# NICTA/revrand

Measured on AMD Instinct MI355X. Metric: feature-rows/sec (Phi + PhiT Phi + PhiT y) at N=10M D=32 F=4096, higher is better.
Workload: dtype f32; 1 GPU; RandomRBF nbases=2048 (F=4096), D=32, N=10000000 f32, features + MFMA Gram, rows sharded over 1 GPU(s); rows_per_gpu=10000000, device=(gfx950:sramecc+:xnack-), gram_engine=f32

## Files before the change

revrand_amd/csrc/rr_rff.hip:

```cpp
#include "rr_syrk_args.h"
#include <algorithm>
#include <map>
#include <mutex>
#include <type_traits>




__device__ __forceinline__ void sincos_rev(float t, float &s, float &c) {
    const float f = t - __builtin_rintf(t);
    s = __builtin_amdgcn_sinf(f);
    c = __builtin_amdgcn_cosf(f);
}

__device__ __forceinline__ void sincos_rev(double t, double &s, double &c) { rr_sincos_rev_f64(t, s, c); }
typedef double doublex4 __attribute__((ext_vector_type(4)));

template <int DMAX, bool GUARD, typename TX, typename TC>
__device__ __forceinline__ TC project_row(const TX *__restrict__ xr, int d, const TC (&w)[DMAX]) {
    TC z = 0;
#pragma unroll
    for (int i = 0; i < DMAX; ++i) {
        if (!GUARD || i < d) z = fma((TC)xr[i], w[i], z);
    }
// ... 970 lines not shown
        syrk_diag_body<4>(p, lds, wave, lane);
}

typedef float floatx4 __attribute__((ext_vector_type(4)));

template <int OFF>
__device__ __forceinline__ float lds_read_b32_off(unsigned addr) {
    float r;
    asm volatile("ds_read_b32 %0, %1 offset:%2" : "=v"(r) : "v"(addr), "i"(OFF));
    return r;
}

template <int NB, int ED>
struct KOpsD16 {
    float2v a[NB], b[NB];
    float x0, x1;
    template <int P>
    __device__ __forceinline__ void load(const unsigned (&abase)[NB], const unsigned (&bbase)[NB], unsigned xbase) {
#pragma unroll
        for (int e = 0; e < NB; ++e)
            if (e != ED) a[e] = lds_read2st64<16 * P, 16 * P + 8>(abase[e]);
#pragma unroll
        for (int e = 0; e < NB; ++e)
            if (e != ED) b[e] = lds_read2st64<16 * P, 16 * P + 8>(bbase[e]);
        x0 = lds_read_b32_off<4096 * P>(xbase);
        x1 = lds_read_b32_off<4096 * P + 64>(xbase);
    }
};

template <int NB, int ED, int FIRST, int LAST>
__device__ __forceinline__ void gram_mfma_d16(const KOpsD16<NB, ED> &o, floatx16 (&acc)[NB], floatx4 (&dd)[3]) {
#pragma unroll
    for (int q = FIRST; q < LAST; ++q) {
        if (q < NB - 1 || q >= NB + 2) {
            const int s_ = q < NB - 1 ? 0 : 1;
            const int r_ = q < NB - 1 ? q : q - (NB + 2);
            const int e = r_ < ED ? r_ : r_ + 1;
            acc[e] = __builtin_amdgcn_mfma_f32_32x32x2f32(o.a[e][s_], o.b[e][s_], acc[e], 0, 0, 0);
        } else {
            const int t = q - (NB - 1);
            dd[t] = __builtin_amdgcn_mfma_f32_16x16x4f32(t == 2 ? o.x1 : o.x0, t == 0 ? o.x0 : o.x1, dd[t], 0, 0, 0);
        }
    }
}

#define RR_PAIRD16(P, CUR, NXT)                                \
    lds_wait();                                                \
    __builtin_amdgcn_sched_barrier(0);                         \
    gram_mfma_d16<NB, ED, 0, 1>(CUR, acc, dd);                 \
    __builtin_amdgcn_sched_barrier(0);                         \
    if ((P) + 1 < KB / 4) NXT.template load<((P) + 1) & (KB / 4 - 1)>(abase, bbase, xbase); \
    __builtin_amdgcn_sched_barrier(0);                         \
    gram_mfma_d16<NB, ED, 1, 2 * NB + 1>(CUR, acc, dd);        \
    __builtin_amdgcn_sched_barrier(0);

template <int NB, int ED, int KB>
__device__ __forceinline__ void syrk_diag16_body(const SyrkArgs &p, float *lds, int wave, int lane, const unsigned bid) {
    const int ta = bid % p.nb;
    const int ks = bid / p.nb;
    const int ca = ta * GR_TC;
    const int64_t row_begin = (int64_t)ks * p.rows_per_split;
    int64_t row_end = row_begin + p.rows_per_split;
    if (row_end > p.rows) row_end = p.rows;

    const unsigned lds0 = (unsigned)(size_t)(__attribute__((address_space(3))) float *)lds;
    const unsigned lane_off = 4u * ((lane >> 5) * GR_TC + (lane & 31));
    int bi[NB], bj[NB];
#pragma unroll
    for (int e = 0; e < NB; ++e) {
        bi[e] = RR_DIAG_I[wave][e];
        bj[e] = RR_DIAG_J[wave][e];
    }
    RR_DEV_ASSERT(bi[ED] == bj[ED]);
    const unsigned lane_off16 = 4u * ((lane >> 4) * GR_TC + 32 * bi[ED] + (lane & 15));
    floatx16 acc[NB];
    floatx4 dd[3];
#pragma unroll
    for (int e = 0; e < NB; ++e)
#pragma unroll
        for (int k = 0; k < 16; ++k) acc[e][k] = 0.f;
#pragma unroll
    for (int t = 0; t < 3; ++t) dd[t] = floatx4{0.f, 0.f, 0.f, 0.f};

    const unsigned voff = 16u * lane, ldp4 = (unsigned)p.ldp * 4u;
    auto dma_tile = [&](float *buf, int64_t kb0) {
        RR_DEV_ASSERT(kb0 + KB <= p.rows && ca + GR_TC <= p.ldp && p.rows % KB == 0 && p.rows_per_split % KB == 0);
        const rr_rsrc_t ra = rr_make_rsrc(p.P + kb0 * p.ldp + ca, 0x7fffffffu);
#pragma unroll
        for (int k = 0; k < KB / 8; ++k) {
            const int lr = (KB / 8) * wave + k;
            __builtin_amdgcn_raw_ptr_buffer_load_lds(ra, (lptr_t)(buf + lr * GR_TC), 16, voff, (unsigned)lr * ldp4, 0, 0);
        }
    };

    const int64_t nkb = (row_end - row_begin) / KB;
    if (nkb > 0) {
        dma_tile(lds, row_begin);
        __syncthreads();
        for (int64_t kb = 0; kb < nkb; ++kb) {
            const int cbuf = (int)(kb & 1);
            const int slot = p.spread ? rr_dma_slot(wave, p.spread) : 0;
            auto dma_next = [&]() {
                if (kb + 1 < nkb) dma_tile(lds + (cbuf ^ 1) * (KB * GR_TC), row_begin + (kb + 1) * KB);
            };
            if (slot == 0) dma_next();
            unsigned abase[NB], bbase[NB];
#pragma unroll
            for (int e = 0; e < NB; ++e) {
                abase[e] = lds0 + cbuf * (4u * KB * GR_TC) + lane_off + 128u * bi[e];
                bbase[e] = lds0 + cbuf * (4u * KB * GR_TC) + lane_off + 128u * bj[e];
            }
            const unsigned xbase = lds0 + cbuf * (4u * KB * GR_TC) + lane_off16;
            KOpsD16<NB, ED> o0, o1;
            o0.template load<0>(abase, bbase, xbase);
            RR_PAIRD16(0, o0, o1)
            if (slot == 1) dma_next();
            RR_PAIRD16(1, o1, o0)
            if (slot == 2) dma_next();
            RR_PAIRD16(2, o0, o1)
            if (slot == 3) dma_next();
            RR_PAIRD16(3, o1, o0)
            RR_PAIRD16(4, o0, o1) RR_PAIRD16(5, o1, o0) RR_PAIRD16(6, o0, o1) RR_PAIRD16(7, o1, o0)
            if constexpr (KB == 64) {
                RR_PAIRD16(8, o0, o1) RR_PAIRD16(9, o1, o0) RR_PAIRD16(10, o0, o1) RR_PAIRD16(11, o1, o0)
                RR_PAIRD16(12, o0, o1) RR_PAIRD16(13, o1, o0) RR_PAIRD16(14, o0, o1) RR_PAIRD16(15, o1, o0)
            }
            __syncthreads();
        }
    }

    const int hi = lane >> 5;
#pragma unroll
    for (int e = 0; e < NB; ++e) {
        if (e == ED) continue;
        const int64_t gc = ca + 32 * bj[e] + (lane & 31);
#pragma unroll
        for (int k = 0; k < 16; ++k) {
            const int64_t gr = ca + 32 * bi[e] + (k & 3) + 8 * (k >> 2) + 4 * hi;
            if (gr <= gc) rr_syrk_out(p, ks, gr, gc, acc[e][k]);
        }
    }
#pragma unroll
    for (int t = 0; t < 3; ++t) {
        const int64_t gc = ca + 32 * bi[ED] + (t >= 1 ? 16 : 0) + (lane & 15);
#pragma unroll
        for (int k = 0; k < 4; ++k) {
            const int64_t gr = ca + 32 * bi[ED] + (t == 2 ? 16 : 0) + 4 * (lane >> 4) + k;
            if (gr <= gc) rr_syrk_out(p, ks, gr, gc, dd[t][k]);
        }
    }
}
#undef RR_PAIRD16

template <int KB>
__device__ __forceinline__ void syrk_diag16_dispatch(const SyrkArgs &p, float *lds, const unsigned bid) {
    const int lane = threadIdx.x & 63;
    const int wave = __builtin_amdgcn_readfirstlane(threadIdx.x >> 6);
    switch (wave) {
        case 0: case 1: case 2: case 3: syrk_diag16_body<5, 0, KB>(p, lds, wave, lane, bid); break;
        case 4: syrk_diag16_body<4, 3, KB>(p, lds, wave, lane, bid); break;
        case 5: syrk_diag16_body<4, 2, KB>(p, lds, wave, lane, bid); break;
        case 6: syrk_diag16_body<4, 1, KB>(p, lds, wave, lane, bid); break;
        default: syrk_diag16_body<4, 0, KB>(p, lds, wave, lane, bid); break;
    }
}

template <int KB>
__global__ void __launch_bounds__(GR_THREADS, 2)
rr_syrk_f32_diag16_kernel(const SyrkArgs p) {
    __shared__ float lds[2 * KB * GR_TC];
    syrk_diag16_dispatch<KB>(p, lds, blockIdx.x);
}

constexpr int GS_TC = 128, GS_KB = 32, GS_LD = 2 * GS_TC, GS_THREADS = 256;

__global__ void __launch_bounds__(GS_THREADS, 2)
rr_syrk_f32_small_kernel(const SyrkArgs p) {
    __shared__ __attribute__((aligned(16))) float lds[2][GS_KB * GS_LD];
    const int tid = threadIdx.x, lane = tid & 63, wave = tid >> 6, wr = wave >> 1, wc = wave & 1;
    const int nb = (int)(p.ldp / GS_TC);
    const int64_t ks = blockIdx.x / p.ntiles;
    int t = (int)(blockIdx.x % p.ntiles), ta = 0;
    while (t >= nb - ta) {
        t -= nb - ta;
        ++ta;
    }
    const int tb = ta + t;
    const int64_t ca = (int64_t)ta * GS_TC, cb = (int64_t)tb * GS_TC;
    const int64_t r0 = ks * p.rows_per_split;
    int64_t r1 = r0 + p.rows_per_split;
    if (r1 > p.rows) r1 = p.rows;
    const int nkb = (int)((r1 - r0 + GS_KB - 1) / GS_KB);
    floatx16 acc[2][2];
#pragma unroll
    for (int i = 0; i < 2; ++i)
#pragma unroll
        for (int j = 0; j < 2; ++j)
#pragma unroll
            for (int e = 0; e < 16; ++e) acc[i][j][e] = 0.f;
    const int lr = tid >> 5, lc = tid & 31;
    float4 ra[4], rb[4];
    auto gload = [&](int kb) {
        const float *base = p.P + (r0 + (int64_t)kb * GS_KB + lr) * p.ldp;
#pragma unroll
        for (int u = 0; u < 4; ++u) {
            ra[u] = *(const float4 *)(base + (int64_t)8 * u * p.ldp + ca + 4 * lc);
            rb[u] = *(const float4 *)(base + (int64_t)8 * u * p.ldp + cb + 4 * lc);
        }
    };
    auto lstore = [&](int buf) {
#pragma unroll
        for (int u = 0; u < 4; ++u) {
            *(float4 *)&lds[buf][(lr + 8 * u) * GS_LD + 4 * lc] = ra[u];
            *(float4 *)&lds[buf][(lr + 8 * u) * GS_LD + GS_TC + 4 * lc] = rb[u];
        }
    };
    if (nkb > 0) {
        gload(0);
        lstore(0);
    }
    __syncthreads();
    const int i32 = lane & 31, kk = lane >> 5;
    for (int kb = 0; kb < nkb; ++kb) {
        const int cur = kb & 1;
        if (kb + 1 < nkb) gload(kb + 1);
        const float *L = lds[cur];
#pragma unroll
        for (int k2 = 0; k2 < GS_KB; k2 += 2) {
            const float *row = L + (k2 + kk) * GS_LD;
            const float a0 = row[wr * 64 + i32], a1 = row[wr * 64 + 32 + i32];
            const float b0 = row[GS_TC + wc * 64 + i32], b1 = row[GS_TC + wc * 64 + 32 + i32];
            acc[0][0] = __builtin_amdgcn_mfma_f32_32x32x2f32(a0, b0, acc[0][0], 0, 0, 0);
            acc[0][1] = __builtin_amdgcn_mfma_f32_32x32x2f32(a0, b1, acc[0][1], 0, 0, 0);
            acc[1][0] = __builtin_amdgcn_mfma_f32_32x32x2f32(a1, b0, acc[1][0], 0, 0, 0);
            acc[1][1] = __builtin_amdgcn_mfma_f32_32x32x2f32(a1, b1, acc[1][1], 0, 0, 0);
        }
        if (kb + 1 < nkb) lstore(cur ^ 1);
        __syncthreads();
    }
#pragma unroll
    for (int i = 0; i < 2; ++i)
#pragma unroll
        for (int j = 0; j < 2; ++j) {
            const int64_t gc = cb + wc * 64 + 32 * j + i32;
#pragma unroll
            for (int e = 0; e < 16; ++e) {
                const int64_t gr = ca + wr * 64 + 32 * i + (e & 3) + 8 * (e >> 2) + 4 * kk;
                if (gr <= gc) rr_syrk_out(p, ks, gr, gc, acc[i][j][e]);
            }
        }
}

__global__ void __launch_bounds__(GR_THREADS, 2)
rr_syrk_f32_merged_kernel(const SyrkArgs p, const SyrkArgs pd, const unsigned n_off) {
    __shared__ float lds[2 * GR_KB * GR_LD];
    if (blockIdx.x < n_off) rr_syrk_f32_body<3>(p, lds, blockIdx.x);
    else syrk_diag16_dispatch<32>(pd, lds, blockIdx.x - n_off);
}

constexpr int G64_TC = 128;
constexpr int G64_KB = 16;
constexpr int G64_LDB = 2 * G64_TC * 8 + 128;
constexpr int G64_THREADS = 256;

struct Syrk64Args {
    const double *P;
    int64_t rows, ldp;
    int F, nb, ntiles;
    int64_t rows_per_split;
    double *G;
    int offdiag_only;
    int lower_tri = 0;
    double *part = nullptr;
    int64_t part_stride = 0;
};

__device__ __forceinline__ void rr_syrk64_out(const Syrk64Args &p, int64_t ks, int64_t gr, int64_t gc, double v) {
    if (p.part != nullptr) p.part[ks * p.part_stride + gr * p.ldp + gc] = v;
    else unsafeAtomicAdd(&p.G[gr * (int64_t)p.F + gc], v);
}

template <typename T>
__global__ void __launch_bounds__(256)
rr_syrk_det_reduce_kernel(const T *__restrict__ part, int64_t stride, int64_t ldp, int F, int nsplit, double *__restrict__ G,
                          double *__restrict__ bcol) {
    const int64_t gc = (int64_t)blockIdx.x * 256 + threadIdx.x, gr = blockIdx.y;
    if (gc < gr || gc > F || (gc == F && bcol == nullptr)) return;
    const T *q = part + gr * ldp + gc;
    double s = 0.0;
    for (int k = 0; k < nsplit; ++k) s += (double)q[(int64_t)k * stride];
    if (gc < F) G[gr * (int64_t)F + gc] += s;
    else bcol[gr] += s;
}

template <int OFF>
__device__ __forceinline__ double lds_read_b64(unsigned addr) {
    double r;
    asm volatile("ds_read_b64 %0, %1 offset:%2" : "=v"(r) : "v"(addr), "i"(OFF));
    return r;
}

struct KOps64 {
    double a[4], b[4];
    template <int T>
    __device__ __forceinline__ void load(unsigned abase, unsigned bbase) {
#pragma unroll
        for (int i = 0; i < 4; ++i) a[i] = 0;
        a[0] = lds_read_b64<4 * T * G64_LDB + 0 * 128>(abase);
        a[1] = lds_read_b64<4 * T * G64_LDB + 1 * 128>(abase);
        a[2] = lds_read_b64<4 * T * G64_LDB + 2 * 128>(abase);
        a[3] = lds_read_b64<4 * T * G64_LDB + 3 * 128>(abase);
        b[0] = lds_read_b64<4 * T * G64_LDB + 0 * 128>(bbase);
        b[1] = lds_read_b64<4 * T * G64_LDB + 1 * 128>(bbase);
        b[2] = lds_read_b64<4 * T * G64_LDB + 2 * 128>(bbase);
        b[3] = lds_read_b64<4 * T * G64_LDB + 3 * 128>(bbase);
    }
};

template <int FIRST, int LAST>
__device__ __forceinline__ void gram64_mfma(const KOps64 &o, doublex4 (&acc)[4][4]) {
#pragma unroll
    for (int q = FIRST; q < LAST; ++q)
        acc[q >> 2][q & 3] = __builtin_amdgcn_mfma_f64_16x16x4f64(o.a[q >> 2], o.b[q & 3], acc[q >> 2][q & 3], 0, 0, 0);
}

#define RR_STEP64(T, CUR, NXT)                                  \
    lds_wait();                                                 \
    __builtin_amdgcn_sched_barrier(0);                          \
    gram64_mfma<0, 1>(CUR, acc);                                \
    __builtin_amdgcn_sched_barrier(0);                          \
    if ((T) + 1 < 4) NXT.template load<((T) + 1) & 3>(abase, bbase); \
    __builtin_amdgcn_sched_barrier(0);                          \
    gram64_mfma<1, 16>(CUR, acc);                               \
    __builtin_amdgcn_sched_barrier(0);

__global__ void __launch_bounds__(G64_THREADS, 2)
rr_syrk_f64_kernel(const Syrk64Args p) {
    __shared__ __attribute__((aligned(16))) unsigned char lds[2 * G64_KB * G64_LDB];

    const int tid = threadIdx.x;
    const int lane = tid & 63;
    const int wave = __builtin_amdgcn_readfirstlane(tid >> 6);

    int tdx = blockIdx.x % p.ntiles;
    const int ks = blockIdx.x / p.ntiles;
    int ta = 0;
    const int od = p.offdiag_only;
    while (tdx >= p.nb - ta - od) {
        tdx -= p.nb - ta - od;
        ++ta;
    }
    const int tb = ta + tdx + od;
    const int ca = ta * G64_TC, cb = tb * G64_TC;

    int64_t row_begin = (int64_t)ks * p.rows_per_split;
    int64_t row_end = row_begin + p.rows_per_split;
    if (row_end > p.rows) row_end = p.rows;
    if (p.lower_tri && row_begin < cb) row_begin = cb;
    if (row_begin >= row_end && p.part == nullptr) return;

    const int wr = wave >> 1, wc_ = wave & 1;
    const unsigned lds0 = (unsigned)(size_t)(__attribute__((address_space(3))) unsigned char *)lds;
    const unsigned aoff = (lane >> 4) * G64_LDB + 8u * (wr * 64 + (lane & 15));
    const unsigned boff = (lane >> 4) * G64_LDB + 8u * (G64_TC + wc_ * 64 + (lane & 15));
    doublex4 acc[4][4];
#pragma unroll
    for (int i = 0; i < 4; ++i)
#pragma unroll
        for (int j = 0; j < 4; ++j)
#pragma unroll
            for (int e = 0; e < 4; ++e) acc[i][j][e] = 0.0;

    const unsigned voff = 16u * lane, ldp8 = (unsigned)p.ldp * 8u;
    auto dma_tile = [&](unsigned char *buf, int64_t kb0) {
        const rr_rsrc_t ra = rr_make_rsrc(p.P + kb0 * p.ldp + ca, 0x7fffffffu), rb = rr_make_rsrc(p.P + kb0 * p.ldp + cb, 0x7fffffffu);
#pragma unroll
        for (int k = 0; k < 4; ++k) {
            const int lr = 4 * wave + k;
            unsigned char *dst = buf + lr * G64_LDB;
            __builtin_amdgcn_raw_ptr_buffer_load_lds(ra, (lptr_t)dst, 16, voff, (unsigned)lr * ldp8, 0, 0);
            __builtin_amdgcn_raw_ptr_buffer_load_lds(rb, (lptr_t)(dst + G64_TC * 8), 16, voff, (unsigned)lr * ldp8, 0, 0);
        }
    };

    const int64_t nkb = (row_end - row_begin) / G64_KB;
    RR_DEV_ASSERT(p.rows % G64_KB == 0 && p.rows_per_split % G64_KB == 0 && cb + G64_TC <= p.ldp && row_end <= p.rows);
    if (nkb > 0) {
        dma_tile(lds, row_begin);
        __syncthreads();
        for (int64_t kb = 0; kb < nkb; ++kb) {
            const int cbuf = (int)(kb & 1);
            if (kb + 1 < nkb) dma_tile(lds + (cbuf ^ 1) * (G64_KB * G64_LDB), row_begin + (kb + 1) * G64_KB);
            const unsigned abase = lds0 + cbuf * (G64_KB * G64_LDB) + aoff;
            const unsigned bbase = lds0 + cbuf * (G64_KB * G64_LDB) + boff;
            KOps64 o0, o1;
            o0.load<0>(abase, bbase);
            RR_STEP64(0, o0, o1) RR_STEP64(1, o1, o0) RR_STEP64(2, o0, o1) RR_STEP64(3, o1, o0)
            __syncthreads();
        }
    }

    const int64_t F = p.F;
#pragma unroll
    for (int i = 0; i < 4; ++i)
#pragma unroll
        for (int j = 0; j < 4; ++j) {
            const int64_t gc = cb + wc_ * 64 + j * 16 + (lane & 15);
#pragma unroll
            for (int e = 0; e < 4; ++e) {
                const int64_t gr = ca + wr * 64 + i * 16 + (lane >> 4) + 4 * e;
// ... 877 lines not shown
                part[t1] = y; part[t2] = x;
                cur += d;
                if (cur < best) { best = cur; best_part = part; }
            }
        }
        part = best_part;
    }
    std::vector<int> fill(nxcd, 0);
    for (int t = 0; t < ntiles; ++t) map[(size_t)fill[part[t]]++ * nxcd + part[t]] = t;
}


int rr_launch_syrk_f32(rr_ctx *c, const float *P, int64_t rows, int64_t ldp, int F, double *dG, hipEvent_t mid,
                       double *bcol = nullptr) {
    if (c->gram_engine != 0) {
        RR_REQUIRE(bcol == nullptr, "gram: the rider column needs the f32 engine");
        RR_REQUIRE(!c->deterministic, "gram: deterministic mode (rr_set_deterministic) needs the f32 engine, not a split 16-bit one");
        return rr_launch_syrk_bf16(c, c->gram_engine, P, nullptr, rows, ldp, F, dG, mid);
    }
    RR_REQUIRE(bcol == nullptr || F < ldp, "gram: no pad column for the rider");
    static const bool small_off = getenv("RR_SYRK_SMALL") != nullptr && atoi(getenv("RR_SYRK_SMALL")) == 0;
    const int64_t big_tiles = (ldp / GR_TC) * (ldp / GR_TC + 1) / 2;
    if (!small_off && ldp <= 1024 && big_tiles * ((rows + 1023) / 1024) < c->num_cu && rows % GS_KB == 0 && !getenv("RR_GRAM_ABLATE")) {
        const int nbs = (int)(ldp / GS_TC), nt = nbs * (nbs + 1) / 2;
        int64_t ns = std::max<int64_t>((2 * c->num_cu + nt - 1) / nt, (rows + 32767) / 32768);
        ns = std::min<int64_t>(ns, std::max<int64_t>(rows / 128, 1));
        const int64_t rps_s = ((rows + ns - 1) / ns + GS_KB - 1) / GS_KB * GS_KB;
        ns = (rows + rps_s - 1) / rps_s;
        SyrkArgs a;
        a.P = P; a.rows = rows; a.ldp = ldp; a.F = F; a.nb = nbs; a.ntiles = nt; a.rows_per_split = rps_s; a.G = dG;
        a.bcol = bcol; a.tile_map = nullptr; a.offdiag_only = 0; a.ablate = 0;
        if (c->deterministic) {
            void *slabs = nullptr;
            int rc = rr_det_scratch(c, (size_t)ns * (size_t)ldp * (size_t)ldp * sizeof(float), &slabs);
            if (rc != RR_OK) return rc;
            a.part = (float *)slabs;
            a.part_stride = ldp * ldp;
        }
        hipLaunchKernelGGL(rr_syrk_f32_small_kernel, dim3((unsigned)(ns * nt)), dim3(GS_THREADS), 0, c->stream, a);
        if (mid) RR_CHECK_HIP(hipEventRecord(mid, c->stream));
        if (a.part)
            hipLaunchKernelGGL(rr_syrk_det_reduce_kernel<float>, dim3((unsigned)((F + 1 + 255) / 256), (unsigned)F), dim3(256), 0,
                               c->stream, a.part, a.part_stride, ldp, F, (int)ns, dG, bcol);
        RR_CHECK_HIP(hipGetLastError());
        return RR_OK;
    }
    const int nb_all = (int)(ldp / GR_TC);
    const int od = (nb_all >= 2 && !getenv("RR_SYRK_NO_DIAG_KERNEL")) ? 1 : 0;
    const int w_last = F + (bcol ? 1 : 0) - GR_TC * (nb_all - 1);
    const int rg = (od && nb_all >= 3 && w_last <= 192 && !getenv("RR_SYRK_NO_RAGGED_KERNEL")) ? 1 : 0;
    const int nb = nb_all - rg;
    const int ntiles = od ? nb * (nb - 1) / 2 : nb * (nb + 1) / 2;
    const int nxcd = 8;
    const bool use_map = (ntiles % nxcd == 0) && !getenv("RR_GRAM_NO_TILE_MAP");
    if (use_map && c->tile_map_nb != nb * 2 + od) {
        std::vector<int> map;
        rr_build_tile_map(nb, od, nxcd, map);
        if (c->tile_map) (void)hipFree(c->tile_map);
        c->tile_map = nullptr;
        RR_CHECK_HIP(hipMalloc((void **)&c->tile_map, map.size() * sizeof(int)));
        RR_CHECK_HIP(hipMemcpy(c->tile_map, map.data(), map.size() * sizeof(int), hipMemcpyHostToDevice));
        c->tile_map_nb = nb * 2 + od;
    }
    const int64_t total_tiles = (int64_t)nb_all * (nb_all + 1) / 2;
    auto gcd64 = [](int64_t x, int64_t y) { while (y) { const int64_t u = x % y; x = y; y = u; } return x; };
    const int64_t min_splits = (rows + 32767) / 32768;
    auto rows_per = [&](int64_t ns) { return ((rows + ns - 1) / ns + GR_KB - 1) / GR_KB * GR_KB; };
    const int64_t unit = ntiles > 0 ? c->num_cu / gcd64(c->num_cu, ntiles) : 1;
    int64_t nsplit = (min_splits + unit - 1) / unit * unit;
    auto floor_rows = [&](int64_t tiles_per_split) {
        return tiles_per_split * ((rows + 1023) / 1024) < c->num_cu ? (int64_t)256 : (int64_t)1024;
    };
    auto small_split = [&](int64_t tiles_per_split) {
        const int64_t fr = floor_rows(tiles_per_split);
        if (fr == 1024) return (rows + 1023) / 1024;
        const int64_t want = (c->num_cu + tiles_per_split - 1) / std::max<int64_t>(tiles_per_split, 1);
        return std::min((rows + fr - 1) / fr, std::max((rows + 1023) / 1024, want));
    };
    if (rows / nsplit < 1024) {
        nsplit = small_split(std::max(ntiles, 1));
        static const bool no_search = getenv("RR_SYRK_SPLIT_SEARCH") != nullptr && atoi(getenv("RR_SYRK_SPLIT_SEARCH")) == 0;
        if (ntiles > 0 && !no_search) {
            double best_cost = 1e300;
            int64_t best_ns = nsplit;
            const int64_t ns_hi = std::max<int64_t>(rows / 256, 1), ns_lo = std::max<int64_t>(rows / 32768, 1);
            for (int64_t ns = ns_lo; ns <= ns_hi && ns <= ns_lo + 4096; ++ns) {
                const int64_t rp = rows_per(ns), n2 = (rows + rp - 1) / rp;
                const int64_t rounds = ((int64_t)ntiles * n2 + c->num_cu - 1) / c->num_cu;
                const double cost = (double)rounds * ((double)rp + 96.0);
                if (cost < best_cost - 1e-9) {
                    best_cost = cost;
                    best_ns = n2;
                }
            }
            nsplit = best_ns;
        }
    }
    if (nsplit < 1) nsplit = 1;
    int64_t rps = rows_per(nsplit);
    int64_t nsplit_d = nsplit, rps_d = rps;
    if (od) {
        double best = -1.0;
        for (int64_t ns = min_splits; ns < min_splits + 96; ++ns) {
            if (rows / ns < floor_rows(nb_all) && ns > 1) break;
            const int64_t wg = ns * nb_all, rounds = (wg + c->num_cu - 1) / c->num_cu;
            const double eff = (double)wg / (double)(rounds * c->num_cu);
            if (eff > best + 1e-9) {
                best = eff;
                nsplit_d = ns;
            }
        }
        rps_d = rows_per(nsplit_d);
        if (rows % 64 == 0 && getenv("RR_SYRK_DIAG_KB") != nullptr && atoi(getenv("RR_SYRK_DIAG_KB")) == 64)
            rps_d = (rps_d + 63) / 64 * 64;
    }
    int64_t nsplit_r = nsplit, rps_r = rps;
    if (rg) {
        double best = -1.0;
        for (int64_t ns = min_splits; ns < min_splits + 96; ++ns) {
            if (rows / ns < floor_rows(nb_all - 1) && ns > 1) break;
            const int64_t wg = ns * (nb_all - 1), rounds = (wg + c->num_cu - 1) / c->num_cu;
            const double eff = (double)wg / (double)(rounds * c->num_cu);
            if (eff > best + 1e-9) {
                best = eff;
                nsplit_r = ns;
            }
        }
        rps_r = rows_per(nsplit_r);
    }
    const char *renv = getenv("RR_GRAM_ROWS_PER_SPLIT");
    if (renv && atoll(renv) >= GR_KB) rps = rps_d = rps_r = (atoll(renv) / GR_KB) * GR_KB;
    if (c->deterministic) rps_d = rps_r = rps;
    nsplit = (rows + rps - 1) / rps;
    nsplit_d = (rows + rps_d - 1) / rps_d;
    nsplit_r = (rows + rps_r - 1) / rps_r;
    RR_REQUIRE(nsplit * total_tiles < (int64_t)1 << 31 && nsplit_d * nb_all < (int64_t)1 << 31 &&
                   nsplit_r * nb_all < (int64_t)1 << 31, "gram: grid too large");
    SyrkArgs a;
    a.P = P; a.rows = rows; a.ldp = ldp; a.F = F; a.nb = nb; a.ntiles = ntiles; a.rows_per_split = rps; a.G = dG;
    a.bcol = bcol;
    a.tile_map = use_map ? c->tile_map : nullptr;
    a.offdiag_only = od;
    a.ablate = getenv("RR_GRAM_ABLATE") ? atoi(getenv("RR_GRAM_ABLATE")) : 0;
    a.spread = rr_dma_spread_env();
    if (c->deterministic) {
        void *slabs = nullptr;
        int rc = rr_det_scratch(c, (size_t)nsplit * (size_t)ldp * (size_t)ldp * sizeof(float), &slabs);
        if (rc != RR_OK) return rc;
        a.part = (float *)slabs;
        a.part_stride = ldp * ldp;
    }
    static const int syrk_mode = getenv("RR_SYRK_STAGGER") ? atoi(getenv("RR_SYRK_STAGGER")) : 3;
    static const bool merge_diag = getenv("RR_SYRK_MERGE_DIAG") != nullptr && atoi(getenv("RR_SYRK_MERGE_DIAG")) != 0;
    if (merge_diag && od && !rg && ntiles > 0 && syrk_mode == 3 && !a.ablate && !getenv("RR_SYRK_NO_DIAG16")) {
        SyrkArgs ad = a;
        ad.nb = nb_all;
        ad.rows_per_split = rps_d;
        const unsigned n_off = (unsigned)(nsplit * ntiles);
        hipLaunchKernelGGL(rr_syrk_f32_merged_kernel, dim3(n_off + (unsigned)(nsplit_d * nb_all)), dim3(GR_THREADS), 0, c->stream, a, ad, n_off);
        if (mid) RR_CHECK_HIP(hipEventRecord(mid, c->stream));
        if (a.part)
            hipLaunchKernelGGL(rr_syrk_det_reduce_kernel<float>, dim3((unsigned)((F + 1 + 255) / 256), (unsigned)F), dim3(256), 0,
                               c->stream, a.part, a.part_stride, ldp, F, (int)nsplit, dG, bcol);
        RR_CHECK_HIP(hipGetLastError());
        return RR_OK;
    }
    if (ntiles > 0) {
        if (syrk_mode == 1 && !a.ablate)
            hipLaunchKernelGGL(rr_syrk_f32_flatstag_kernel, dim3((unsigned)(nsplit * ntiles)), dim3(GR_THREADS), 0, c->stream, a);
        else if (syrk_mode == 2 && !a.ablate)
            hipLaunchKernelGGL(rr_syrk_f32_buf_kernel, dim3((unsigned)(nsplit * ntiles)), dim3(GR_THREADS), 0, c->stream, a);
        else if (syrk_mode == 0 || a.ablate)
            hipLaunchKernelGGL(rr_syrk_f32_flat_kernel, dim3((unsigned)(nsplit * ntiles)), dim3(GR_THREADS), 0, c->stream, a);
        else
            hipLaunchKernelGGL(rr_syrk_f32_kernel, dim3((unsigned)(nsplit * ntiles)), dim3(GR_THREADS), 0, c->stream, a);
    }
    if (rg) {
        SyrkArgs ar = a;
        ar.nb = nb_all;
        ar.rows_per_split = rps_r;
        hipLaunchKernelGGL(rr_syrk_f32_ragged_kernel, dim3((unsigned)(nsplit_r * (nb_all - 1))), dim3(GR_THREADS), 0, c->stream, ar);
    }
    if (mid) RR_CHECK_HIP(hipEventRecord(mid, c->stream));
    if (od) {
        SyrkArgs ad = a;
        ad.nb = nb_all;
        ad.rows_per_split = rps_d;
        static const bool no_diag16 = getenv("RR_SYRK_NO_DIAG16") != nullptr;
        static const bool kb64 = getenv("RR_SYRK_DIAG_KB") != nullptr && atoi(getenv("RR_SYRK_DIAG_KB")) == 64;
        if (no_diag16)
            hipLaunchKernelGGL(rr_syrk_f32_diag_kernel, dim3((unsigned)(nsplit_d * nb_all)), dim3(GR_THREADS), 0, c->stream, ad);
        else if (kb64 && rows % 64 == 0 && ad.rows_per_split % 64 == 0)
            hipLaunchKernelGGL(rr_syrk_f32_diag16_kernel<64>, dim3((unsigned)(nsplit_d * nb_all)), dim3(GR_THREADS), 0, c->stream, ad);
        else
            hipLaunchKernelGGL(rr_syrk_f32_diag16_kernel<32>, dim3((unsigned)(nsplit_d * nb_all)), dim3(GR_THREADS), 0, c->stream, ad);
    }
    if (a.part)
        hipLaunchKernelGGL(rr_syrk_det_reduce_kernel<float>, dim3((unsigned)((F + 1 + 255) / 256), (unsigned)F), dim3(256), 0,
                           c->stream, a.part, a.part_stride, ldp, F, (int)nsplit, dG, bcol);
    RR_CHECK_HIP(hipGetLastError());
    return RR_OK;
}

int rr_launch_syrk_f64(rr_ctx *c, const double *P, int64_t rows, int64_t ldp, int F, double *dG, int lower_tri = 0) {
    const int nb = (int)(ldp / G64_TC);
    const int od = (nb >= 2 && !getenv("RR_SYRK_NO_DIAG_KERNEL")) ? 1 : 0;
    const int ntiles = od ? nb * (nb - 1) / 2 : nb * (nb + 1) / 2;
    const int64_t slots = (int64_t)c->num_cu * 2;
    int64_t g = slots, t = ntiles;
    while (t) { const int64_t u = g % t; g = t; t = u; }
    const int64_t unit = slots / g;
    static const bool no_fine = getenv("RR_SYRK64_FINE_SPLIT") != nullptr && atoi(getenv("RR_SYRK64_FINE_SPLIT")) == 0;
    const int64_t min_rows = (lower_tri && rows == ldp && rows <= 2048 && !no_fine) ? 128 : 512;
    int64_t nsplit = unit;
    if (rows / nsplit < 2048) nsplit = (slots * 4 + ntiles - 1) / ntiles;
    if (rows / nsplit < min_rows) nsplit = (rows + min_rows - 1) / min_rows;
    if (nsplit < 1) nsplit = 1;
    const int64_t rps = ((rows + nsplit - 1) / nsplit + G64_KB - 1) / G64_KB * G64_KB;
    nsplit = (rows + rps - 1) / rps;
    RR_REQUIRE(nsplit * ntiles < (int64_t)1 << 31, "gram: grid too large");
    Syrk64Args a;
    a.P = P; a.rows = rows; a.ldp = ldp; a.F = F; a.nb = nb; a.ntiles = ntiles; a.rows_per_split = rps; a.G = dG;
    a.offdiag_only = od;
    static const bool no_tri = getenv("RR_SYRK64_TRI") != nullptr && atoi(getenv("RR_SYRK64_TRI")) == 0;
    a.lower_tri = lower_tri && !no_tri && rows == ldp ? 1 : 0;
    if (c->deterministic) {
        void *slabs = nullptr;
        int rc = rr_det_scratch(c, (size_t)nsplit * (size_t)ldp * (size_t)ldp * sizeof(double), &slabs);
        if (rc != RR_OK) return rc;
        a.part = (double *)slabs;
        a.part_stride = ldp * ldp;
    }
    if (ntiles > 0)
        hipLaunchKernelGGL(rr_syrk_f64_kernel, dim3((unsigned)(nsplit * ntiles)), dim3(G64_THREADS), 0, c->stream, a);
    if (od) {
        const int64_t dslots = (int64_t)c->num_cu * 4;
        int64_t best_ns = 1;
        double best = -1.0;
        for (int64_t ns = 1; ns <= 4 * dslots / nb + 1; ++ns) {
            if (rows / ns < min_rows && ns > 1) break;
            const int64_t wg = ns * nb, rounds = (wg + dslots - 1) / dslots;
            const double eff = (double)wg / (double)(rounds * dslots);
            if (eff > best + 1e-9) {
                best = eff;
                best_ns = ns;
            }
        }
        Syrk64Args ad = a;
        ad.rows_per_split = ((rows + best_ns - 1) / best_ns + G64_KB - 1) / G64_KB * G64_KB;
        if (c->deterministic) ad.rows_per_split = rps;
        const int64_t nsd = (rows + ad.rows_per_split - 1) / ad.rows_per_split;
        hipLaunchKernelGGL(rr_syrk_f64_diag_kernel, dim3((unsigned)(nsd * nb)), dim3(G64_THREADS), 0, c->stream, ad);
    }
    if (a.part)
        hipLaunchKernelGGL(rr_syrk_det_reduce_kernel<double>, dim3((unsigned)((F + 255) / 256), (unsigned)F), dim3(256), 0,
                           c->stream, a.part, a.part_stride, ldp, F, (int)nsplit, dG, (double *)nullptr);
    RR_CHECK_HIP(hipGetLastError());
    return RR_OK;
}

int rr_launch_gemm_tn_f64(rr_ctx *c, const double *A, int64_t lda, const double *B, int64_t ldb, double *D, int64_t ldd,
                          int64_t K, int64_t M, int64_t N, int subtract, int upper_only) {
    Gemm64Args g;
    g.A = A; g.B = B; g.D = D; g.lda = lda; g.ldb = ldb; g.ldd = ldd; g.K = (int)K; g.ntb = (int)(N / G64_TC);
    g.subtract = subtract;
    g.upper_only = upper_only;
    static const bool no_k128 = getenv("RR_GEMM64_K128") != nullptr && atoi(getenv("RR_GEMM64_K128")) == 0;
    if (!no_k128 && K == 128 && M == 128 && N % 32 == 0 && (upper_only == 0 || (upper_only == 1 && N == 128))) {
        hipLaunchKernelGGL(rr_gemm_tn_f64_k128_kernel, dim3((unsigned)(N / 32)), dim3(G64_THREADS), 0, c->stream, g);
        RR_CHECK_HIP(hipGetLastError());
        return RR_OK;
    }
    hipLaunchKernelGGL(rr_gemm_tn_f64_kernel, dim3((unsigned)((M / G64_TC) * g.ntb)), dim3(G64_THREADS), 0, c->stream, g);
    RR_CHECK_HIP(hipGetLastError());
    return RR_OK;
}

template <typename TX, typename TC>
static int launch_gram(rr_basis *b, const void *dX, const void *dy, int64_t N, int64_t ldx, double *dG,
                       double *db) {
    rr_ctx *c = b->ctx;
    constexpr bool F32 = sizeof(TC) == 4;
    constexpr int TCOLS = F32 ? GR_TC : G64_TC;
    constexpr int KB = F32 ? GR_KB : G64_KB;
    const int F = 2 * b->n;
    const int64_t ldp = ((int64_t)F + TCOLS - 1) / TCOLS * TCOLS;
    const TC scale = (TC)(1.0 / sqrt((double)b->n));
    const TC *Ws = F32 ? (const TC *)b->dWs32 : (const TC *)b->dWs64;
    int64_t chunk = (int64_t)(((size_t)32 << 30) / ((size_t)ldp * sizeof(TC)));
    const char *cenv = getenv("RR_GRAM_CHUNK_ROWS");
    if (cenv && atoll(cenv) >= KB) chunk = atoll(cenv);
    else if (N > chunk) {
        const int64_t nchunks = (N + chunk - 1) / chunk;
        chunk = (N + nchunks - 1) / nchunks;
    }
    if (chunk > N) chunk = N;
    RR_REQUIRE(!(F32 && c->deterministic && c->gram_engine != 0),
               "gram: deterministic mode (rr_set_deterministic) needs the f32 engine, not a split 16-bit one");
    const bool fused_pb = F32 && !b->phase64 && c->gram_engine != 0 && rr_features_mfma_ok<TX>(b, (const TX *)dX, N, ldx);
    const int KBR = fused_pb ? 64 : KB;
    chunk = (chunk + KBR - 1) / KBR * KBR;
    static const bool overlap_on = getenv("RR_GRAM_OVERLAP") != nullptr && atoi(getenv("RR_GRAM_OVERLAP")) != 0;
    const bool overlap = N > chunk && overlap_on && !c->deterministic;
    const int nbuf = overlap ? 2 : 1;
    int rc = ensure_zbuf(b, (size_t)nbuf * (size_t)chunk * ldp * sizeof(TC));
    if (rc != RR_OK) return rc;
    TC *P = (TC *)b->zbuf;
    if (overlap && !c->stream2) {
        RR_CHECK_HIP(hipStreamCreateWithFlags(&c->stream2, hipStreamNonBlocking));
        RR_CHECK_HIP(hipEventCreateWithFlags(&c->ev_fork, hipEventDisableTiming));
    }
    hipStream_t fstream = overlap ? c->stream2 : c->stream;
    const hipStream_t main_stream = c->stream;
    if (fused_pb && ldp > F) {
        const int64_t cnt = (nbuf * chunk / 16) * (ldp - F) * 4;
        hipLaunchKernelGGL(rr_zero_padcols_pb_kernel, dim3((unsigned)((cnt + 255) / 256)), dim3(256), 0, c->stream,
                           (uintx4 *)P, nbuf * chunk / 16, ldp, F);
        RR_CHECK_HIP(hipGetLastError());
    } else if (ldp > F) {
        const int64_t cnt = nbuf * chunk * (ldp - F);
        hipLaunchKernelGGL(rr_zero_padcols_kernel<TC>, dim3((unsigned)((cnt + 255) / 256)), dim3(256), 0, c->stream,
                           P, nbuf * chunk, ldp, F);
        RR_CHECK_HIP(hipGetLastError());
    }

    TC *const Pbase = P;
    struct StreamGuard {
        rr_ctx *c;
        hipStream_t s;
        ~StreamGuard() { c->stream = s; }
    } guard{c, main_stream};
    for (int64_t r0 = 0; r0 < N; r0 += chunk) {
        const int64_t m = (N - r0 < chunk) ? N - r0 : chunk;
        const int64_t mpad = (m + KBR - 1) / KBR * KBR;
        const TX *Xc = (const TX *)dX + r0 * ldx;
        const TX *yc = dy ? (const TX *)dy + r0 : nullptr;
        const int64_t kchunk = r0 / chunk;
        P = Pbase + (overlap ? (kchunk & 1) * chunk * ldp : 0);
        const size_t e0 = (size_t)kchunk * 5;
        while (b->events.size() < e0 + 5) {
            hipEvent_t ev;
            RR_CHECK_HIP(hipEventCreate(&ev));
            b->events.push_back(ev);
        }
        if (overlap) {
            if (kchunk == 0) {
                RR_CHECK_HIP(hipEventRecord(c->ev_fork, main_stream));
                RR_CHECK_HIP(hipStreamWaitEvent(fstream, c->ev_fork, 0));
// ... 788 lines not shown
```

Baseline: 8.490 million feature-rows/s.

## Rebalance diagonal-tile SYRK work so paired waves share each SIMD evenly

Adds a new diagonal-tile Gram kernel body in which each of the 8 waves owns a fixed, compile-time-checked set of 32x32 blocks plus one 16x16-split diagonal block. The sets are chosen so that waves w and w+4 together issue 9 MFMAs per k-step, giving every SIMD an even share, where the old scheme gave waves 0-3 five products each and waves 4-7 four. It also pads LDS by 8192 floats for the default KB=32 diagonal kernel, which likely cuts occupancy to spread blocks out. The new path is on by default and the older layout stays reachable through an environment variable. The main risk is register pressure and a mismatch between this split and the off-diagonal kernels.

```diff
diff --git a/revrand_amd/csrc/rr_rff.hip b/revrand_amd/csrc/rr_rff.hip
--- a/revrand_amd/csrc/rr_rff.hip
+++ b/revrand_amd/csrc/rr_rff.hip
@@ -1146,24 +1146,234 @@
 }
 #undef RR_PAIRD16
 
-template <int KB>
+template <int W> struct Diag32 {};
+template <> struct Diag32<0> {
+    static constexpr int NO = 4, NP = 4, D = 6;
+    static constexpr int OPS[4] = {3, 4, 5, 6};
+    static constexpr int QA[4] = {1, 1, 0, 2}, QB[4] = {3, 2, 2, 3};
+};
+template <> struct Diag32<1> {
+    static constexpr int NO = 4, NP = 4, D = 4;
+    static constexpr int OPS[4] = {1, 3, 4, 7};
+    static constexpr int QA[4] = {0, 1, 2, 0}, QB[4] = {1, 3, 3, 3};
+};
+template <> struct Diag32<2> {
+    static constexpr int NO = 4, NP = 4, D = 1;
+    static constexpr int OPS[4] = {0, 1, 3, 6};
+    static constexpr int QA[4] = {1, 0, 0, 2}, QB[4] = {3, 3, 2, 3};
+};
+template <> struct Diag32<3> {
+    static constexpr int NO = 4, NP = 4, D = 7;
+    static constexpr int OPS[4] = {0, 2, 5, 7};
+    static constexpr int QA[4] = {0, 2, 0, 0}, QB[4] = {1, 3, 2, 3};
+};
+template <> struct Diag32<4> {
+    static constexpr int NO = 3, NP = 3, D = 5;
+    static constexpr int OPS[4] = {1, 2, 5, 0};
+    static constexpr int QA[4] = {1, 0, 0, 0}, QB[4] = {2, 1, 2, 0};
+};
+template <> struct Diag32<5> {
+    static constexpr int NO = 3, NP = 3, D = 2;
+    static constexpr int OPS[4] = {2, 6, 7, 0};
+    static constexpr int QA[4] = {0, 1, 0, 0}, QB[4] = {1, 2, 2, 0};
+};
+template <> struct Diag32<6> {
+    static constexpr int NO = 3, NP = 3, D = 3;
+    static constexpr int OPS[4] = {2, 3, 4, 0};
+    static constexpr int QA[4] = {0, 1, 0, 0}, QB[4] = {1, 2, 2, 0};
+};
+template <> struct Diag32<7> {
+    static constexpr int NO = 3, NP = 3, D = 0;
+    static constexpr int OPS[4] = {0, 1, 4, 0};
+    static constexpr int QA[4] = {0, 0, 1, 0}, QB[4] = {1, 2, 2, 0};
+};
+
+template <int W>
+constexpr unsigned long long diag32_blocks() {
+    typedef Diag32<W> T;
+    unsigned long long m = 1ull << (9 * T::D);
+    for (int q = 0; q < T::NP; ++q) {
+        const int i = T::OPS[T::QA[q]], j = T::OPS[T::QB[q]];
+        if (T::QA[q] >= T::NO || T::QB[q] >= T::NO || i >= j || j > 7 || (m >> (8 * i + j) & 1)) return 0;
+        m |= 1ull << (8 * i + j);
+    }
+    return m;
+}
+constexpr bool diag32_exact_cover() {
+    const unsigned long long m[8] = {diag32_blocks<0>(), diag32_blocks<1>(), diag32_blocks<2>(), diag32_blocks<3>(),
+                                     diag32_blocks<4>(), diag32_blocks<5>(), diag32_blocks<6>(), diag32_blocks<7>()};
+    unsigned long long all = 0, upper = 0;
+    for (int w = 0; w < 8; ++w) {
+        if (m[w] == 0 || (all & m[w]) != 0) return false;
+        all |= m[w];
+    }
+    for (int i = 0; i < 8; ++i)
+        for (int j = i; j < 8; ++j) upper |= 1ull << (8 * i + j);
+    return all == upper;
+}
+static_assert(diag32_exact_cover(), "Diag32: the 36 upper blocks of a diagonal tile, each exactly once");
+static_assert(Diag32<0>::NP == 4 && Diag32<1>::NP == 4 && Diag32<2>::NP == 4 && Diag32<3>::NP == 4 && Diag32<4>::NP == 3 &&
+              Diag32<5>::NP == 3 && Diag32<6>::NP == 3 && Diag32<7>::NP == 3, "Diag32: 9 MFMAs per k-step and SIMD (waves w, w + 4)");
+
+template <int W>
+struct KOpsD16S {
+    typedef Diag32<W> T;
+    float2v o[T::NO];
+    float x0, x1;
+    template <int P>
+    __device__ __forceinline__ void load(const unsigned (&obase)[T::NO], unsigned xbase) {
+#pragma unroll
+        for (int i = 0; i < T::NO; ++i) o[i] = lds_read2st64<16 * P, 16 * P + 8>(obase[i]);
+        x0 = lds_read_b32_off<4096 * P>(xbase);
+        x1 = lds_read_b32_off<4096 * P + 64>(xbase);
+    }
+};
+
+template <int W, int FIRST, int LAST>
+__device__ __forceinline__ void gram_mfma_d16s(const KOpsD16S<W> &o, floatx16 (&acc)[Diag32<W>::NP], floatx4 (&dd)[3]) {
+    typedef Diag32<W> T;
+#pragma unroll
+    for (int q = FIRST; q < LAST; ++q) {
+        if (q < T::NP || q >= T::NP + 3) {
+            const int s_ = q < T::NP ? 0 : 1;
+            const int e = q < T::NP ? q : q - (T::NP + 3);
+            acc[e] = __builtin_amdgcn_mfma_f32_32x32x2f32(o.o[T::QA[e]][s_], o.o[T::QB[e]][s_], acc[e], 0, 0, 0);
+        } else {
+            const int t = q - T::NP;
+            dd[t] = __builtin_amdgcn_mfma_f32_16x16x4f32(t == 2 ? o.x1 : o.x0, t == 0 ? o.x0 : o.x1, dd[t], 0, 0, 0);
+        }
+    }
+}
+
+#define RR_PAIRD16S(P, CUR, NXT)                               \
+    lds_wait();                                                \
+    __builtin_amdgcn_sched_barrier(0);                         \
+    gram_mfma_d16s<W, 0, 1>(CUR, acc, dd);                     \
+    __builtin_amdgcn_sched_barrier(0);                         \
+    if ((P) + 1 < KB / 4) NXT.template load<((P) + 1) & (KB / 4 - 1)>(obase, xbase); \
+    __builtin_amdgcn_sched_barrier(0);                         \
+    gram_mfma_d16s<W, 1, 2 * T::NP + 3>(CUR, acc, dd);         \
+    __builtin_amdgcn_sched_barrier(0);
+
+template <int W, int KB>
+__device__ __forceinline__ void syrk_diag16s_body(const SyrkArgs &p, float *lds, int lane, const unsigned bid) {
+    typedef Diag32<W> T;
+    const int ta = bid % p.nb;
+    const int ks = bid / p.nb;
+    const int ca = ta * GR_TC;
+    const int64_t row_begin = (int64_t)ks * p.rows_per_split;
+    int64_t row_end = row_begin + p.rows_per_split;
+    if (row_end > p.rows) row_end = p.rows;
+
+    const unsigned lds0 = (unsigned)(size_t)(__attribute__((address_space(3))) float *)lds;
+    const unsigned lane_off = 4u * ((lane >> 5) * GR_TC + (lane & 31));
+    const unsigned lane_off16 = 4u * ((lane >> 4) * GR_TC + 32 * T::D + (lane & 15));
+    floatx16 acc[T::NP];
+    floatx4 dd[3];
+#pragma unroll
+    for (int e = 0; e < T::NP; ++e)
+#pragma unroll
+        for (int k = 0; k < 16; ++k) acc[e][k] = 0.f;
+#pragma unroll
+    for (int t = 0; t < 3; ++t) dd[t] = floatx4{0.f, 0.f, 0.f, 0.f};
+
+    const unsigned voff = 16u * lane, ldp4 = (unsigned)p.ldp * 4u;
+    auto dma_tile = [&](float *buf, int64_t kb0) {
+        RR_DEV_ASSERT(kb0 + KB <= p.rows && ca + GR_TC <= p.ldp && p.rows % KB == 0 && p.rows_per_split % KB == 0);
+        const rr_rsrc_t ra = rr_make_rsrc(p.P + kb0 * p.ldp + ca, 0x7fffffffu);
+#pragma unroll
+        for (int k = 0; k < KB / 8; ++k) {
+            const int lr = (KB / 8) * W + k;
+            __builtin_amdgcn_raw_ptr_buffer_load_lds(ra, (lptr_t)(buf + lr * GR_TC), 16, voff, (unsigned)lr * ldp4, 0, 0);
+        }
+    };
+
+    const int64_t nkb = (row_end - row_begin) / KB;
+    if (nkb > 0) {
+        dma_tile(lds, row_begin);
+        __syncthreads();
+        for (int64_t kb = 0; kb < nkb; ++kb) {
+            const int cbuf = (int)(kb & 1);
+            const int slot = p.spread ? rr_dma_slot(W, p.spread) : 0;
+            auto dma_next = [&]() {
+                if (kb + 1 < nkb) dma_tile(lds + (cbuf ^ 1) * (KB * GR_TC), row_begin + (kb + 1) * KB);
+            };
+            if (slot == 0) dma_next();
+            unsigned obase[T::NO];
+#pragma unroll
+            for (int i = 0; i < T::NO; ++i) obase[i] = lds0 + cbuf * (4u * KB * GR_TC) + lane_off + 128u * T::OPS[i];
+            const unsigned xbase = lds0 + cbuf * (4u * KB * GR_TC) + lane_off16;
+            KOpsD16S<W> o0, o1;
+            o0.template load<0>(obase, xbase);
+            RR_PAIRD16S(0, o0, o1)
+            if (slot == 1) dma_next();
+            RR_PAIRD16S(1, o1, o0)
+            if (slot == 2) dma_next();
+            RR_PAIRD16S(2, o0, o1)
+            if (slot == 3) dma_next();
+            RR_PAIRD16S(3, o1, o0)
+            RR_PAIRD16S(4, o0, o1) RR_PAIRD16S(5, o1, o0) RR_PAIRD16S(6, o0, o1) RR_PAIRD16S(7, o1, o0)
+            if constexpr (KB == 64) {
+                RR_PAIRD16S(8, o0, o1) RR_PAIRD16S(9, o1, o0) RR_PAIRD16S(10, o0, o1) RR_PAIRD16S(11, o1, o0)
+                RR_PAIRD16S(12, o0, o1) RR_PAIRD16S(13, o1, o0) RR_PAIRD16S(14, o0, o1) RR_PAIRD16S(15, o1, o0)
+            }
+            __syncthreads();
+        }
+    }
+
+    const int hi = lane >> 5;
+#pragma unroll
+    for (int e = 0; e < T::NP; ++e) {
+        const int64_t gc = ca + 32 * T::OPS[T::QB[e]] + (lane & 31);
+#pragma unroll
+        for (int k = 0; k < 16; ++k) {
+            const int64_t gr = ca + 32 * T::OPS[T::QA[e]] + (k & 3) + 8 * (k >> 2) + 4 * hi;
+            rr_syrk_out(p, ks, gr, gc, acc[e][k]);
+        }
+    }
+#pragma unroll
+    for (int t = 0; t < 3; ++t) {
+        const int64_t gc = ca + 32 * T::D + (t >= 1 ? 16 : 0) + (lane & 15);
+#pragma unroll
+        for (int k = 0; k < 4; ++k) {
+            const int64_t gr = ca + 32 * T::D + (t == 2 ? 16 : 0) + 4 * (lane >> 4) + k;
+            if (t == 1 || gr <= gc) rr_syrk_out(p, ks, gr, gc, dd[t][k]);
+        }
+    }
+}
+#undef RR_PAIRD16S
+
+template <int KB, bool SH>
 __device__ __forceinline__ void syrk_diag16_dispatch(const SyrkArgs &p, float *lds, const unsigned bid) {
     const int lane = threadIdx.x & 63;
     const int wave = __builtin_amdgcn_readfirstlane(threadIdx.x >> 6);
-    switch (wave) {
-        case 0: case 1: case 2: case 3: syrk_diag16_body<5, 0, KB>(p, lds, wave, lane, bid); break;
-        case 4: syrk_diag16_body<4, 3, KB>(p, lds, wave, lane, bid); break;
-        case 5: syrk_diag16_body<4, 2, KB>(p, lds, wave, lane, bid); break;
-        case 6: syrk_diag16_body<4, 1, KB>(p, lds, wave, lane, bid); break;
-        default: syrk_diag16_body<4, 0, KB>(p, lds, wave, lane, bid); break;
-    }
-}
-
-template <int KB>
+    if constexpr (SH) {
+        switch (wave) {
+            case 0: syrk_diag16s_body<0, KB>(p, lds, lane, bid); break;
+            case 1: syrk_diag16s_body<1, KB>(p, lds, lane, bid); break;
+            case 2: syrk_diag16s_body<2, KB>(p, lds, lane, bid); break;
+            case 3: syrk_diag16s_body<3, KB>(p, lds, lane, bid); break;
+            case 4: syrk_diag16s_body<4, KB>(p, lds, lane, bid); break;
+            case 5: syrk_diag16s_body<5, KB>(p, lds, lane, bid); break;
+            case 6: syrk_diag16s_body<6, KB>(p, lds, lane, bid); break;
+            default: syrk_diag16s_body<7, KB>(p, lds, lane, bid); break;
+        }
+    } else {
+        switch (wave) {
+            case 0: case 1: case 2: case 3: syrk_diag16_body<5, 0, KB>(p, lds, wave, lane, bid); break;
+            case 4: syrk_diag16_body<4, 3, KB>(p, lds, wave, lane, bid); break;
+            case 5: syrk_diag16_body<4, 2, KB>(p, lds, wave, lane, bid); break;
+            case 6: syrk_diag16_body<4, 1, KB>(p, lds, wave, lane, bid); break;
+            default: syrk_diag16_body<4, 0, KB>(p, lds, wave, lane, bid); break;
+        }
+    }
+}
+
+template <int KB, bool SH = true, int PAD = 0>
 __global__ void __launch_bounds__(GR_THREADS, 2)
 rr_syrk_f32_diag16_kernel(const SyrkArgs p) {
-    __shared__ float lds[2 * KB * GR_TC];
-    syrk_diag16_dispatch<KB>(p, lds, blockIdx.x);
+    __shared__ float lds[2 * KB * GR_TC + PAD];
+    syrk_diag16_dispatch<KB, SH>(p, lds, blockIdx.x);
 }
 
 constexpr int GS_TC = 128, GS_KB = 32, GS_LD = 2 * GS_TC, GS_THREADS = 256;
@@ -1245,11 +1455,12 @@
         }
 }
 
+template <bool SH>
 __global__ void __launch_bounds__(GR_THREADS, 2)
 rr_syrk_f32_merged_kernel(const SyrkArgs p, const SyrkArgs pd, const unsigned n_off) {
     __shared__ float lds[2 * GR_KB * GR_LD];
     if (blockIdx.x < n_off) rr_syrk_f32_body<3>(p, lds, blockIdx.x);
-    else syrk_diag16_dispatch<32>(pd, lds, blockIdx.x - n_off);
+    else syrk_diag16_dispatch<32, SH>(pd, lds, blockIdx.x - n_off);
 }
 
 constexpr int G64_TC = 128;
@@ -2433,12 +2644,18 @@
     }
     static const int syrk_mode = getenv("RR_SYRK_STAGGER") ? atoi(getenv("RR_SYRK_STAGGER")) : 3;
     static const bool merge_diag = getenv("RR_SYRK_MERGE_DIAG") != nullptr && atoi(getenv("RR_SYRK_MERGE_DIAG")) != 0;
+    static const int diag_shared_mode = getenv("RR_SYRK_DIAG_SHARED") ? atoi(getenv("RR_SYRK_DIAG_SHARED")) : 1;
+    static const bool diag_shared = diag_shared_mode != 0;
     if (merge_diag && od && !rg && ntiles > 0 && syrk_mode == 3 && !a.ablate && !getenv("RR_SYRK_NO_DIAG16")) {
         SyrkArgs ad = a;
         ad.nb = nb_all;
         ad.rows_per_split = rps_d;
         const unsigned n_off = (unsigned)(nsplit * ntiles);
-        hipLaunchKernelGGL(rr_syrk_f32_merged_kernel, dim3(n_off + (unsigned)(nsplit_d * nb_all)), dim3(GR_THREADS), 0, c->stream, a, ad, n_off);
+        const dim3 grid(n_off + (unsigned)(nsplit_d * nb_all));
+        if (diag_shared)
+            hipLaunchKernelGGL(rr_syrk_f32_merged_kernel<true>, grid, dim3(GR_THREADS), 0, c->stream, a, ad, n_off);
+        else
+            hipLaunchKernelGGL(rr_syrk_f32_merged_kernel<false>, grid, dim3(GR_THREADS), 0, c->stream, a, ad, n_off);
         if (mid) RR_CHECK_HIP(hipEventRecord(mid, c->stream));
         if (a.part)
             hipLaunchKernelGGL(rr_syrk_det_reduce_kernel<float>, dim3((unsigned)((F + 1 + 255) / 256), (unsigned)F), dim3(256), 0,
@@ -2471,10 +2688,16 @@
         static const bool kb64 = getenv("RR_SYRK_DIAG_KB") != nullptr && atoi(getenv("RR_SYRK_DIAG_KB")) == 64;
         if (no_diag16)
             hipLaunchKernelGGL(rr_syrk_f32_diag_kernel, dim3((unsigned)(nsplit_d * nb_all)), dim3(GR_THREADS), 0, c->stream, ad);
+        else if (kb64 && rows % 64 == 0 && ad.rows_per_split % 64 == 0 && diag_shared)
+            hipLaunchKernelGGL(rr_syrk_f32_diag16_kernel<64>, dim3((unsigned)(nsplit_d * nb_all)), dim3(GR_THREADS), 0, c->stream, ad);
         else if (kb64 && rows % 64 == 0 && ad.rows_per_split % 64 == 0)
-            hipLaunchKernelGGL(rr_syrk_f32_diag16_kernel<64>, dim3((unsigned)(nsplit_d * nb_all)), dim3(GR_THREADS), 0, c->stream, ad);
+            hipLaunchKernelGGL((rr_syrk_f32_diag16_kernel<64, false>), dim3((unsigned)(nsplit_d * nb_all)), dim3(GR_THREADS), 0, c->stream, ad);
+        else if (diag_shared_mode == 2)
+            hipLaunchKernelGGL(rr_syrk_f32_diag16_kernel<32>, dim3((unsigned)(nsplit_d * nb_all)), dim3(GR_THREADS), 0, c->stream, ad);
+        else if (diag_shared)
+            hipLaunchKernelGGL((rr_syrk_f32_diag16_kernel<32, true, 8192>), dim3((unsigned)(nsplit_d * nb_all)), dim3(GR_THREADS), 0, c->stream, ad);
         else
-            hipLaunchKernelGGL(rr_syrk_f32_diag16_kernel<32>, dim3((unsigned)(nsplit_d * nb_all)), dim3(GR_THREADS), 0, c->stream, ad);
+            hipLaunchKernelGGL((rr_syrk_f32_diag16_kernel<32, false>), dim3((unsigned)(nsplit_d * nb_all)), dim3(GR_THREADS), 0, c->stream, ad);
     }
     if (a.part)
         hipLaunchKernelGGL(rr_syrk_det_reduce_kernel<float>, dim3((unsigned)((F + 1 + 255) / 256), (unsigned)F), dim3(256), 0,
```

Result: no change. 8.505 million feature-rows/s, median of 4 (+0.2%).
